# obah/zk-research-implementations

Hardware: AMD Instinct MI355X
Metric: GKR sum-check field-ops/sec + prover ms, 24-var BN254, 1/2/4/8 GPU (higher is better)
Workload: dtype u256 mod p (8x32-bit Montgomery limbs)

## Files before the change

zk-research-implementations_amd/csrc/gkr_plan.hpp:

```cpp
#pragma once
#include <stddef.h>
#include <stdint.h>

#include <vector>

#if defined(__HIPCC__)
#define ZK_PLAN_HD __host__ __device__ __forceinline__
#else
#define ZK_PLAN_HD static inline
#endif

namespace zk {
ZK_PLAN_HD uint64_t tail_region(uint64_t h0, uint32_t m) { return 8 * (h0 - (h0 >> m)); }
ZK_PLAN_HD uint64_t dtail_region(uint64_t Q0, uint32_t s) {
  uint64_t o = 0;
  for (uint32_t t = 0; t < s; ++t) o += 16 * (Q0 >> (2 * t));
  return o;
}
}

namespace zkh {
struct GStep {
  int kind;
  uint32_t i;
  int np;
  uint32_t nd = 0;
  bool dfs = false;
};
enum {
  GS_ROUND0 = 0, GS_SINGLE = 1, GS_DOUBLE = 2, GS_TAIL = 3, GS_DTAIL = 4, GS_D0 = 5, GS_D0T = 6, GS_T32 = 7, GS_T33 = 8,
  GS_HOST = 11
};
inline uint32_t rounds_of(const GStep& st, uint32_t nv) {
  switch (st.kind) {
    case GS_DOUBLE: case GS_D0: case GS_T32: return 2;
    case GS_D0T: case GS_T33: return 3;
    case GS_DTAIL: return 2 * st.nd;
    case GS_TAIL: case GS_HOST: return nv - st.i;
    default: return 1;
  }
}

struct PlanKnobs {
  bool pre = true;
  bool dround = true, d0 = true, d0t = true, dtail = true;
  bool use_tail = true;
  bool cross_ranks = false;
  bool device_fs = false;
  uint64_t dtail_max_quads = 1u << 10, tail_max_pairs = 1u << 15;
  uint32_t host_rounds = 4;
  uint32_t num_cus = 256, t33_oct64_min = 1, mall_order = 0;
};

struct PhasePlan {
  std::vector<GStep> steps;
  uint32_t stop = 0;
  uint32_t host_rounds = 0;
  uint32_t d0t_order = 0;
  uint64_t tail_elems = 0;
  size_t host_tab_bytes = 0;
  bool fslog = false;
  const char* error = nullptr;
};

inline PhasePlan plan_phase(const PlanKnobs& k, uint32_t nv, bool host_ok, uint32_t gather_max) {
  PhasePlan pl;
  std::vector<GStep>& steps = pl.steps;
  const uint64_t L = (uint64_t)1 << nv;
  const bool d0t = k.dround && k.d0t && nv >= 11;
  int nt = -1;
  if (d0t)
    for (int q = 0; 3 + 3 * q + 8 <= (int)nv; ++q) {
      const int R = (int)nv - 3 - 3 * q;
      if (R % 2 == 0 && (R >= 12 || nt < 0)) nt = q;
    }
  const bool d0t_doubles = d0t && nt >= 0;
  const bool d0 = !d0t_doubles && k.dround && k.d0 && nv >= 2 && nv % 2 == 0;
  const bool persistent = k.pre && k.use_tail;
  if (nv >= 1) steps.push_back({d0t_doubles ? GS_D0T : (d0 ? GS_D0 : GS_ROUND0), 0, 0});
  if (d0t_doubles) {
    for (int q = 0; q < nt; ++q) steps.push_back({GS_T33, 3u + 3u * q, 3});
    steps.push_back({GS_T32, 3u + 3u * nt, 3});
  }
  if (k.dround) {
    uint32_t i = d0t_doubles ? 5u + 3u * nt : (d0 ? 2 : 1);
    int np = d0t_doubles || d0 ? 2 : 1;
    if (!d0 && !d0t_doubles) {
      if (nv >= 2) steps.push_back({GS_SINGLE, i++, 0});
      if (nv >= 3 && (nv - 2) % 2 == 1) steps.push_back({GS_SINGLE, i++, 0});
    }
    for (; i + 1 < nv; i += 2, np = 2) steps.push_back({GS_DOUBLE, i, np});
    auto small = [&](const GStep& st) { return st.kind == GS_DOUBLE && (L >> st.i) / 4 <= k.dtail_max_quads; };
    if (host_ok && persistent && k.dtail && !k.cross_ranks && k.host_rounds >= 2) {
      for (uint32_t H = k.host_rounds & ~1u; H >= 2 && pl.host_rounds == 0; H -= 2) {
        size_t e = steps.size();
        uint32_t got = 0;
        while (got < H && e > 0 && steps[e - 1].kind == GS_DOUBLE && steps[e - 1].np == 2) {
          --e;
          got += 2;
        }
        size_t smalls = 0;
        for (size_t q = 0; q < e; ++q) smalls += small(steps[q]);
        if (got == H && smalls >= 2 && e == steps.size() - H / 2) {
          steps.resize(e);
          pl.host_rounds = H;
// ... 78 lines not shown
```

zk-research-implementations_amd/csrc/gkr_rounds.hpp:

```cpp
#pragma once
#include <stddef.h>
#include <stdint.h>
#include <string.h>

#include <vector>

#include "hfield.hpp"
#include "keccak.hpp"

using zk::Fe;

struct zk_transcript {
  zk::Keccak256 h;
};

namespace zkh {
template <class F>
void canon_bytes(const Fe& m, uint8_t out[32]) {
  const Fe c = zk::hfe_from_mont<F>(m);
  memcpy(out, c.v, 32);
}
template <class F>
Fe challenge(zk_transcript* t) {
  uint8_t d[32];
// ... 155 lines not shown
  for (int b = 0; b < 3; ++b) {
    V[b] = fe_zero<F>();
    for (int a = 0; a < 3; ++a)
      V[b] = hfe_add<F>(V[b], hfe_mul<F>(wa[a], hfe_add<F>(T[9 * a + 3 * b], T[9 * a + 3 * b + 1])));
  }
  later_round<F>(s, i0 + 1, V[0], at2w(V[0], V[1], V[2]));
  Fe wb[3];
  wts(s.r, wb);
  Fe Z[3];
  for (int g = 0; g < 3; ++g) {
    uint64_t acc[9] = {0};
    for (int a = 0; a < 3; ++a) {
      uint64_t in[9] = {0};
      for (int b = 0; b < 3; ++b) h64::mac_wide(in, h64::of(wb[b]), h64::of(T[9 * a + 3 * b + g]));
      h64::mac_wide(acc, h64::of(wa[a]), h64::of(wide_to_fe<F>(in)));
    }
    Z[g] = wide_to_fe<F>(acc);
  }
  later_round<F>(s, i0 + 2, Z[0], at2w(Z[0], Z[1], Z[2]));
}

template <class F>
void two_rounds(RoundState& s, uint32_t i0, bool first, const Fe* d) {
  using namespace zk;
  const Fe e0 = hfe_add<F>(d[0], d[2]);
  const Fe e1 = first ? hfe_add<F>(d[4], d[8]) : hfe_sub<F>(s.claim, e0);
  one_round<F>(s, i0, e0, e1, hfe_add<F>(d[5], d[6]));
  const Fe &r = s.r, one = fe_one<F>(), two = hfe_add<F>(one, one);
  const Fe rm1 = hfe_sub<F>(r, one), rm2 = hfe_sub<F>(r, two);
  const Fe L0 = hfe_half<F>(hfe_mul<F>(rm1, rm2));
  const Fe L1 = hfe_sub<F>(fe_zero<F>(), hfe_mul<F>(r, rm2));
  const Fe L2 = hfe_half<F>(hfe_mul<F>(r, rm1));
  auto lag = [&](const Fe& v0, const Fe& v1, const Fe& v2) {
    return hfe_add<F>(hfe_add<F>(hfe_mul<F>(L0, v0), hfe_mul<F>(L1, v1)), hfe_mul<F>(L2, v2));
  };
  const Fe f0 = lag(d[0], d[4], d[5]), f2 = lag(d[3], d[7], d[1]);
  later_round<F>(s, i0 + 1, f0, f2);
}

template <class F>
void eq8_weights(const Fe& rz, const Fe& ra, const Fe& rb, Fe (&e)[8]) {
  using namespace zk;
  Fe ab[4];
  ab[3] = hfe_mul<F>(rz, ra);
  ab[2] = hfe_sub<F>(rz, ab[3]);
  ab[1] = hfe_sub<F>(ra, ab[3]);
  ab[0] = hfe_sub<F>(hfe_sub<F>(fe_one<F>(), rz), ab[1]);
  for (int q = 0; q < 4; ++q) {
    e[2 * q + 1] = hfe_mul<F>(ab[q], rb);
    e[2 * q] = hfe_sub<F>(ab[q], e[2 * q + 1]);
  }
}

template <class F>
void host_rounds(RoundState& s, uint32_t i, uint32_t nv, const uint64_t* raw, FinalVals* fin) {
  const size_t len = (size_t)1 << (nv - i + 2);
  std::vector<Fe> T[4];
  for (int t = 0; t < 4; ++t) {
    const uint64_t* w = raw + (size_t)t * 4 * len;
    T[t].resize(len);
    for (size_t e = 0; e < len; ++e)
      for (int k = 0; k < 4; ++k) {
        const uint64_t x = w[k * len + e];
        T[t][e].v[2 * k] = (uint32_t)x;
        T[t][e].v[2 * k + 1] = (uint32_t)(x >> 32);
      }
  }
  host_fold<F>(T, s.ra);
  host_fold<F>(T, s.rb);
  for (; i < nv; ++i) {
    Fe e0, e2;
    host_round_sums<F>(T, e0, e2);
    later_round<F>(s, i, e0, e2);
    if (i + 1 < nv || fin) host_fold<F>(T, s.r);
  }
  if (fin) {
    for (int t = 0; t < 4; ++t) fin->v[t] = T[t][0];
    fin->ok = true;
  }
}

template <class F>
const char* replay_device_fs(RoundState& s, uint32_t i, const uint32_t (*cf)[8], uint32_t m, const uint32_t* rd) {
  using namespace zk;
  if (m > 3) return "device Fiat-Shamir record corrupt";
  Fe c[3];
  for (uint32_t q = 0; q < 3; ++q) {
    if (q < m) memcpy(c[q].v, cf[q], 32);
    else c[q] = fe_zero<F>();
  }
  const Fe s01 = hfe_add<F>(hfe_add<F>(hfe_add<F>(c[0], c[0]), c[1]), c[2]);
  if (memcmp(s01.v, s.claim.v, 32) != 0) return "device Fiat-Shamir round polynomial does not match the running claim";
  s.claim = absorb_round<F>(s.tr, c, (int)m, s.k0 + i, s.out, s.r);
  if (memcmp(s.r.v, rd, 32) != 0) return "device Fiat-Shamir challenge differs from the host transcript";
  s.drew();
  return nullptr;
}
}
```

zk-research-implementations_amd/csrc/host.hpp:

```cpp
#pragma once
#include <hip/hip_runtime.h>
#include <hip/hip_ext.h>
#include <rccl/rccl.h>

#include <algorithm>
#include <chrono>
#include <cstdio>
#include <cstdlib>
#include <cstring>
#include <memory>
#include <new>
#include <string>
#include <utility>
#include <vector>

#include "../../include/zk_sumcheck.h"
#include "field.hpp"
#include "keccak.hpp"
#include "kernels.hpp"
#include "mfma.hpp"
#include "gkr_plan.hpp"
#include "gkr_rounds.hpp"
#include "fft_plan.hpp"
#include "poly_plan.hpp"
// ... 22 lines not shown
  } while (0)

template <class Fn>
int guarded(Fn&& fn) {
  try {
    fn();
    g_last_error.clear();
    return ZK_OK;
  } catch (const ZkError& e) {
    g_last_error = e.msg;
    return e.code;
  } catch (const std::bad_alloc&) {
    g_last_error = "host allocation failed";
    return ZK_ENOMEM;
  } catch (...) {
    g_last_error = "unknown error";
    return ZK_EDEVICE;
  }
}

inline void require(bool cond, const char* msg) {
  if (!cond) fail(ZK_EINVAL, msg);
}

template <class Fn>
void dispatch(zk_field field, Fn&& fn) {
  switch (field) {
    case ZK_BN254_FR: fn(zk::Bn254Fr{}); break;
    case ZK_BN254_FQ: fn(zk::Bn254Fq{}); break;
    case ZK_BLS12_381_FR: fn(zk::Bls12_381Fr{}); break;
    default: fail(ZK_EINVAL, "unknown field");
  }
}

inline Fe from_zk(const zk_fe& a) {
  Fe r;
  memcpy(r.v, a.limb, 32);
  return r;
}
inline zk_fe to_zk(const Fe& a) {
  zk_fe r;
  memcpy(r.limb, a.v, 32);
  return r;
}

template <class F>
Fe in_mont(zk_repr repr, const zk_fe& a) {
  Fe x = from_zk(a);
  require(zk::fe_is_canonical<F>(x), "field element >= modulus");
  return repr == ZK_REPR_MONTGOMERY ? x : zk::fe_to_mont<F>(x);
}
template <class F>
zk_fe out_repr(zk_repr repr, const Fe& m) {
  return to_zk(repr == ZK_REPR_MONTGOMERY ? m : zk::fe_from_mont<F>(m));
}

}
using namespace zkh;

namespace zkh {
struct DevBuf {
  void* p = nullptr;
  size_t bytes = 0;
  void ensure(size_t b) {
    if (b <= bytes) return;
    if (p) HIPCK(hipFree(p));
    p = nullptr;
    bytes = 0;
    if (hipMalloc(&p, b) != hipSuccess) {
      p = nullptr;
      (void)hipGetLastError();
      fail(ZK_ENOMEM, "hipMalloc of " + std::to_string(b) + " bytes failed");
    }
    bytes = b;
  }
  void release() {
    if (p) (void)hipFree(p);
    p = nullptr;
    bytes = 0;
  }
  Fe* fe(size_t off_elems = 0) const { return reinterpret_cast<Fe*>(p) + off_elems; }
};
struct ScopedBuf {
  DevBuf b;
  ScopedBuf() = default;
  ScopedBuf(const ScopedBuf&) = delete;
  ScopedBuf& operator=(const ScopedBuf&) = delete;
  ~ScopedBuf() { b.release(); }
};

struct FftTables {
  int field = 0;
  uint32_t m = 0;
  bool inverse = false;
  uint32_t log_w = 0, h = 0;
  DevBuf stage_roots, hi, lo, lo_scaled;
  Fe n_inv;
};

enum CommKind { COMM_NONE = 0, COMM_HOST = 1, COMM_RCCL = 2 };
}
using namespace zkh;

struct zk_ctx {
  int device = 0;
  int num_cus = 256;
  hipStream_t stream = nullptr;
  DevBuf work[2];
  DevBuf input;
  DevBuf partials;
  DevBuf tailbuf;
  DevBuf small;
  uint64_t* h_red = nullptr;
  uint32_t tag = 0;
  uint64_t lanes_max_pairs = 1u << 15;
  std::chrono::steady_clock::time_point work_t0;
  bool work_open = false;
  uint32_t timing = 0;
  zk_stats stats{};
  struct Pending {
    int kind;
    hipEvent_t a, b;
    double bytes;
  };
  std::vector<zk_launch> launch_log;
  std::vector<std::pair<hipEvent_t, hipEvent_t>> ev_free;
  std::vector<Pending> pending;
  int rank = 0, world = 1;
  CommKind comm = COMM_NONE;
  zk_allreduce_u64_fn ar = nullptr;
  bool force_coll = false;
  bool prelaunch = true;
  bool host_prelaunch = false;
  bool dround = true;
  int d0 = 3;
  bool d0t = true;
  bool dm = true;
  uint64_t dm_min_quads = 1u << 17;
  bool dtail = true;
  uint64_t dtail_max_quads = 1u << 10;
  uint32_t dtail_blocks = 64;
  uint32_t gather_vars = 10;
  DevBuf gbuf;
  bool t33_pipe = true;
  uint32_t lc_loads = 7;
  uint32_t mall_order = 0;
  uint32_t t33_oct64_min = 1;
  uint32_t host_rounds = 4;
  uint64_t* h_tab = nullptr;
  bool device_fs = false;
  zk::FsLog* h_fslog = nullptr;
  size_t h_tab_bytes = 0;
  bool tail = true;
  bool circuit_dense = false;
  uint32_t circuit_host_lgl = 9;
  uint64_t tail_max_pairs = 1u << 15;
  uint64_t* tail_trace = nullptr;
  uint64_t* block_trace = nullptr;
  int block_trace_step = -1;
  uint32_t grid_cap = 0;
  uint32_t atomic_fanin = 1024;
  uint32_t rtag = 0;
  void* user = nullptr;
  ncclComm_t nccl = nullptr;
  bool peer = false;
  uint64_t* peer_buf = nullptr;
  uint64_t* peer_gbuf = nullptr;
  std::vector<void*> peer_open;
  zk::PeerSlots* d_peer = nullptr;
  uint64_t peer_seq = 0;
  DevBuf msm[19];
  bool msm_balanced = true;
  uint32_t msm_win_task = 4;
  DevBuf scan_tmp[4];
  DevBuf g1_table;
  DevBuf g1_table16;
  uint32_t fft_stages = kFftTileLog;
  DevBuf fft_scratch[2];
  std::vector<std::unique_ptr<FftTables>> fft_tables;
  uint32_t poly_host_max = kPolyHostMaxDefault;
  DevBuf poly_scratch[3];
  uint32_t composed_host_lg = zkc::kComposedHostLgDefault;
  std::vector<zk_wired_circuit*> wired;
};


namespace zkh {
constexpr size_t kSmallBytes = 160 * 1024;
constexpr size_t kBlockTraceMax = 8192;
inline uint64_t* d_red(zk_ctx* c) { return reinterpret_cast<uint64_t*>(c->small.p); }
inline uint32_t* d_flag(zk_ctx* c) { return reinterpret_cast<uint32_t*>(reinterpret_cast<char*>(c->small.p) + 2048); }
inline uint32_t* d_counter(zk_ctx* c) { return reinterpret_cast<uint32_t*>(reinterpret_cast<char*>(c->small.p) + 2560); }
inline uint64_t* d_accum(zk_ctx* c) { return reinterpret_cast<uint64_t*>(reinterpret_cast<char*>(c->small.p) + 4096); }
inline char* d_gather(zk_ctx* c) { return reinterpret_cast<char*>(c->small.p) + 8192; }
constexpr size_t kHostPage = 8192;
inline uint32_t* h_flag(zk_ctx* c) { return reinterpret_cast<uint32_t*>(reinterpret_cast<char*>(c->h_red) + 2048); }
inline zk::RWait* h_rin(zk_ctx* c) { return reinterpret_cast<zk::RWait*>(reinterpret_cast<char*>(c->h_red) + 4096); }
inline uint32_t* h_err(zk_ctx* c) { return reinterpret_cast<uint32_t*>(reinterpret_cast<char*>(c->h_red) + 4160); }
inline zk::RPost* h_rpost(zk_ctx* c) { return reinterpret_cast<zk::RPost*>(reinterpret_cast<char*>(c->h_red) + 6144); }
inline zk::RWait* d_relay(zk_ctx* c) { return reinterpret_cast<zk::RWait*>(reinterpret_cast<char*>(c->small.p) + 6144); }
inline zk::RPost* d_rpost(zk_ctx* c) { return reinterpret_cast<zk::RPost*>(reinterpret_cast<char*>(c->small.p) + 6656); }
static_assert(6656 + sizeof(zk::RPost) <= 8192 && 6144 + sizeof(zk::RPost) <= kHostPage, "relay slot overlaps");

inline void bind(zk_ctx* c) { HIPCK(hipSetDevice(c->device)); }
void wired_release_all(zk_ctx* c);
template <class F>
void eq_table_device(zk_ctx* c, const Fe* pt, uint32_t n, Fe* dst, Fe* tmp);
uint32_t kzg_nvars(const zk_kzg* k);
void check_g1_points(const zk_g1* pts, uint32_t n);

template <class K>
uint32_t grid_for(zk_ctx* c, uint64_t work, K kernel) {
  static thread_local std::vector<std::pair<const void*, int>> cache;
  int per_cu = 0;
  for (auto& e : cache)
// ... 386 lines not shown
    const uint64_t t = (uint64_t)tag << 32;
    for (int i = 0; i < 8; ++i) {
      __atomic_store_n(&s->w[24 + i], t | dig[i], __ATOMIC_RELAXED);
      __atomic_store_n(&s->w[32 + i], t | claim.v[i], __ATOMIC_RELAXED);
    }
    post2(ra, rb, rab, tag);
  }
  ~PostR() {
    if (done || last == 0) return;
    post(zk::fe_zero<zk::Bn254Fr>(), last);
    Fe z[8];
    for (auto& x : z) x = zk::fe_zero<zk::Bn254Fr>();
    post8(z, last);
    (void)hipStreamSynchronize(c->stream);
  }
};

inline bool prelaunch(zk_ctx* c, uint32_t nv) {
  return c->prelaunch && nv > 1 && (c->comm != COMM_HOST || c->host_prelaunch);
}

inline bool use_tail(zk_ctx* c, bool across_ranks) {
  return c->tail && !(across_ranks && multi_rank(c) && (c->comm == COMM_RCCL || c->peer));
}
constexpr size_t kTailRelayBytes = 64 * sizeof(zk::RPost);
inline PlanKnobs plan_knobs(zk_ctx* c, uint32_t nv, bool across_ranks) {
  PlanKnobs k;
  k.pre = prelaunch(c, nv);
  k.dround = c->dround;
  k.d0 = c->d0 > 0;
  k.d0t = c->d0t;
  k.dtail = c->dtail;
  k.use_tail = use_tail(c, across_ranks);
  k.cross_ranks = across_ranks && multi_rank(c);
  k.device_fs = c->device_fs;
  k.dtail_max_quads = c->dtail_max_quads;
  k.tail_max_pairs = c->tail_max_pairs;
  k.host_rounds = c->host_rounds;
  k.num_cus = (uint32_t)c->num_cus;
  k.t33_oct64_min = c->t33_oct64_min;
  k.mall_order = c->mall_order;
  return k;
}

inline void prepare_phase_buffers(zk_ctx* c, const PhasePlan& pl) {
  if (pl.fslog && !c->h_fslog) {
    HIPCK(hipHostMalloc(reinterpret_cast<void**>(&c->h_fslog), 64 * sizeof(zk::FsLog),
                        hipHostMallocMapped | hipHostMallocCoherent));
    memset(c->h_fslog, 0, 64 * sizeof(zk::FsLog));
  }
  if (pl.tail_elems > 0) {
    const size_t had = c->tailbuf.bytes;
    c->tailbuf.ensure(kTailRelayBytes + pl.tail_elems * sizeof(Fe));
    if (c->tailbuf.bytes != had) HIPCK(hipMemset(c->tailbuf.p, 0, kTailRelayBytes));
  }
  if (c->h_tab_bytes < pl.host_tab_bytes) {
    if (c->h_tab) HIPCK(hipHostFree(c->h_tab));
    c->h_tab = nullptr;
    c->h_tab_bytes = 0;
    HIPCK(hipHostMalloc(reinterpret_cast<void**>(&c->h_tab), pl.host_tab_bytes, hipHostMallocMapped | hipHostMallocCoherent));
    c->h_tab_bytes = pl.host_tab_bytes;
  }
}

inline zk::DIn make_din(zk_ctx* c, bool pre, uint32_t& rtag, const Fe& ra, const Fe& rb, const Fe& rab) {
  zk::DIn d{};
  if (pre) {
    d.host = h_rpost(c);
    d.relay = d_rpost(c);
    d.err = h_err(c);
    d.tag = rtag = ++c->rtag;
  } else {
    d.ra = ra;
    d.rb = rb;
    d.rab = rab;
  }
  return d;
}
inline zk::RoundIn make_rin(zk_ctx* c, bool pre, uint32_t& rtag, const Fe& r) {
  zk::RoundIn in{};
  if (pre) {
    in.host = h_rin(c);
    in.relay = d_relay(c);
    in.err = h_err(c);
    in.tag = rtag = ++c->rtag;
  } else {
    in.r = r;
  }
  return in;
}

template <class F>
struct PhaseRun {
  zk_ctx* c;
  const Fe** cur;
  uint32_t nv;
  bool across_ranks, pre;
  const PhasePlan& pl;
  FinalVals* fin;
  RoundState rs;
  std::vector<zk::RoundSink> sinks;
  std::vector<uint32_t> rtags;
  int inbuf;
  PostR post;

  void out_tables(uint64_t size, Fe* nx[4]) {
    const int ob = inbuf == 0 ? 1 : 0;
    Fe* w = c->work[ob].fe();
    for (int t = 0; t < 4; ++t) nx[t] = w + (uint64_t)t * size;
    inbuf = ob;
  }
  void wrote(Fe* const nx[4], const zk::RoundSink& sk, int limbs) {
    for (int t = 0; t < 4; ++t) cur[t] = nx[t];
    enqueue_reduce(c, sk, across_ranks, limbs);
  }

  void enqueue_input(const GStep& st) {
    const uint64_t size = (uint64_t)1 << nv, h = size / 2;
    const zk::RoundSink& sk = sinks[0];
    if (st.kind == GS_ROUND0) {
      const uint32_t grid = grid_for(c, 2 * h, zk::k_gkr_round0<F>);
      launch(c, ZK_K_GKR_ROUND0, 256.0 * h, 6.0 * h, zk::k_gkr_round0<F>, grid, cur[0], cur[1], cur[2], cur[3], h, sk);
      enqueue_reduce(c, sk, across_ranks, 3 * 17);
    } else if (st.kind == GS_D0) {
      const uint64_t Q = size / 4, nch = (Q + 31) / 32;
      const uint32_t res = grid_for(c, nch * zk::kBlock, zk::k_gkr_d0m<F>);
      const uint32_t grid = step_grid(c, res, (nch + 2 * zk::kD0MChunksMax - 1) / (2 * zk::kD0MChunksMax));
      launch(c, ZK_K_GKR_D0, 128.0 * size, 4.5 * size, zk::k_gkr_d0m<F>, grid, cur[0], cur[1], cur[2], cur[3], Q, sk);
      enqueue_reduce(c, sk, across_ranks, zk::kD0Limbs);
    } else {
      const uint64_t O = size / 8, nch = O / 32;
      const auto kern = (c->lc_loads & 1u) ? zk::k_gkr_d0t<F, true> : zk::k_gkr_d0t<F>;
      const uint32_t res = grid_for(c, 2 * nch * zk::kBlock, kern) & ~1u;
      const uint32_t grid = step_grid(c, res, std::max<uint64_t>(2, 2 * ((nch + zk::kD0TChunksMax - 1) / zk::kD0TChunksMax))) & ~1u;
      launch(c, ZK_K_GKR_D0, 128.0 * size, 8.0 * size, kern, grid, cur[0], cur[1], cur[2], cur[3], O, pl.d0t_order, sk);
      enqueue_reduce(c, sk, across_ranks, zk::kD0TLimbs);
    }
  }
  void enqueue_by_three(size_t si) {
    const GStep& st = pl.steps[si];
    const uint64_t size = ((uint64_t)1 << nv) >> st.i;
    const zk::RoundSink& sk = sinks[st.i];
    Fe* nx[4];
    out_tables(size, nx);
    const zk::DIn din = make_din(c, pre, rtags[si], rs.rz, rs.ra, rs.rb);
    if (st.kind == GS_T32) {
      const uint64_t Q = size / 4, nch = Q / zk::kDMQuads;
      const uint32_t res = grid_for(c, nch * zk::kBlock, zk::k_gkr_dm3<F>);
      const uint32_t grid = step_grid(c, res, (nch + zk::kDMChunksMax - 1) / zk::kDMChunksMax);
      launch(c, ZK_K_GKR_DM, 4608.0 * Q, 48.0 * Q, zk::k_gkr_dm3<F>, grid, cur[0], cur[1], cur[2], cur[3], nx[0],
             nx[1], nx[2], nx[3], Q, din, sk);
      return wrote(nx, sk, zk::kDLimbs);
    }
    const uint64_t O = size / 8;
    const bool o64 = O / 64 >= (uint64_t)c->num_cus * c->t33_oct64_min;
// ... 109 lines not shown
    switch (st.kind) {
      case GS_ROUND0: case GS_D0: case GS_D0T: return enqueue_input(st);
      case GS_T32: case GS_T33: return enqueue_by_three(si);
      case GS_TAIL: return enqueue_tail(si);
      case GS_DTAIL: return enqueue_dtail(si);
      case GS_DOUBLE: return enqueue_double(si);
      default: return enqueue_single(si);
    }
  }
  uint32_t last_tag(size_t si) const {
    const GStep& st = pl.steps[si];
    return rtags[si] + (st.kind == GS_TAIL ? nv - st.i - 1 : (st.kind == GS_DTAIL ? st.nd - 1 : 0));
  }

  void single(uint32_t i) {
    Fe s2[2];
    collect_sums<F, 2>(c, sinks[i], across_ranks, 17, s2);
    later_round<F>(rs, i, s2[0], s2[1]);
  }
  void two(uint32_t i0) {
    Fe d[zk::kDCats];
    collect_sums<F, zk::kDCats>(c, sinks[i0], across_ranks, 17, d);
    two_rounds<F>(rs, i0, false, d);
  }
  void three(uint32_t i0, bool first) {
    Fe T[zk::kD0TCats];
    collect_sums<F, zk::kD0TCats>(c, sinks[i0], across_ranks, 9, T, true);
    three_rounds<F>(rs, i0, first, T);
  }
  void post_pair(uint32_t tag) { post.post2(rs.ra, rs.rb, zk::hfe_mul<F>(rs.ra, rs.rb), tag); }
  void dtail(size_t si) {
    const GStep& st = pl.steps[si];
    const uint32_t last = st.i + 2 * (st.nd - 1);
    if (!st.dfs) {
      for (uint32_t d = 0; d < st.nd; ++d) {
        two(st.i + 2 * d);
        if (d + 1 < st.nd) post_pair(rtags[si] + d + 1);
      }
      return;
    }
    wait_flag(c, sinks[last].tag);
    for (uint32_t d = 0; d + 1 < st.nd; ++d) {
      const zk::FsLog& lg = c->h_fslog[d];
      if (__atomic_load_n(&lg.tag, __ATOMIC_ACQUIRE) != rtags[si] + d) fail(ZK_EDEVICE, "device Fiat-Shamir record missing");
      for (int j = 0; j < 2; ++j) {
        if (const char* bad = replay_device_fs<F>(rs, st.i + 2 * d + j, lg.c[j], lg.m[j], lg.r[j])) fail(ZK_EDEVICE, bad);
        c->stats.device_fs_rounds += 1;
      }
    }
    two(last);
  }
  void host(const GStep& st) {
    const auto t0 = std::chrono::steady_clock::now();
    std::vector<uint64_t> raw((size_t)16 << (nv - st.i + 2));
    memcpy(raw.data(), c->h_tab, raw.size() * 8);
    const auto t1 = std::chrono::steady_clock::now();
    host_rounds<F>(rs, st.i, nv, raw.data(), fin);
    if (c->tail_trace)
      fprintf(stderr, "zk host rounds %u..%u: %.2f us (table copy %.2f us)\n", st.i, nv - 1,
              std::chrono::duration<double, std::micro>(std::chrono::steady_clock::now() - t0).count(),
              std::chrono::duration<double, std::micro>(t1 - t0).count());
  }
  uint32_t derive(size_t si) {
    const GStep& st = pl.steps[si];
    switch (st.kind) {
      case GS_ROUND0: {
        Fe s3[3];
        collect_sums<F, 3>(c, sinks[0], across_ranks, 17, s3);
        one_round<F>(rs, 0, s3[0], s3[1], s3[2]);
        return 1;
      }
      case GS_D0: {
        Fe d[zk::kD0Cats];
        collect_sums<F, zk::kD0Cats>(c, sinks[0], across_ranks, 17, d);
        two_rounds<F>(rs, 0, true, d);
        return 2;
      }
      case GS_D0T: case GS_T33: three(st.i, st.kind == GS_D0T); return 3;
      case GS_T32: case GS_DOUBLE: two(st.i); return 2;
      case GS_SINGLE: single(st.i); return 1;
      case GS_TAIL:
        for (uint32_t i = st.i; i < nv; ++i) {
          single(i);
          if (pre && i + 1 < nv) post.post(rs.r, rtags[si] + (i + 1 - st.i));
        }
        return 1;
      case GS_HOST: host(st); return 0;
      default: dtail(si); return 2;
    }
  }
  void hand_on(size_t si) {
    if (!pre || si + 1 >= pl.steps.size()) return;
    const GStep& nx = pl.steps[si + 1];
    const uint32_t tag = rtags[si + 1];
    const Fe z = zk::fe_zero<F>();
    if (nx.kind == GS_HOST) return;
    if (nx.kind == GS_T32 || nx.kind == GS_T33) {
      Fe e[8];
      eq8_weights<F>(rs.rz, rs.ra, rs.rb, e);
      post.post8(e, tag);
    } else if (nx.kind == GS_DTAIL && nx.dfs) {
      const zk::Keccak256& h = rs.tr->h;
      bool fresh = h.fill == 32;
      for (int q = 0; q < 25; ++q) fresh = fresh && h.st[q] == 0;
      if (!fresh) fail(ZK_EINVAL, "internal: device Fiat-Shamir needs a transcript right after a challenge");
      uint32_t dig[8];
      memcpy(dig, h.buf, 32);
      const bool two = nx.np == 2;
      post.post5(two ? rs.ra : z, rs.rb, two ? zk::hfe_mul<F>(rs.ra, rs.rb) : z, dig, rs.claim, tag);
    } else if (nx.kind == GS_DOUBLE || nx.kind == GS_DTAIL) {
// ... 41 lines not shown
      auto pr = [](const char* what, std::vector<double> v) {
        if (v.empty()) return;
        std::sort(v.begin(), v.end());
        fprintf(stderr, "    %-22s min %8.2f  p10 %8.2f  med %8.2f  p90 %8.2f  max %8.2f us (%zu blocks)\n", what, v.front(),
                v[v.size() / 10], v[v.size() / 2], v[v.size() * 9 / 10], v.back(), v.size());
      };
      if (const char* fn = getenv("ZK_DEBUG_BLOCKS_FILE")) {
        if (FILE* f = fopen(fn, "w")) {
          fprintf(f, "block,loop_end,fanin_start,counted_in\n");
          for (size_t b = 0; b < kBlockTraceMax; ++b) {
            const uint64_t* q = c->block_trace + 8 * b;
            if (!q[0] || !q[1] || !q[2]) continue;
            fprintf(f, "%zu,%.2f,%.2f,%.2f\n", b, ((int64_t)q[0] - (int64_t)rr) * 0.01, ((int64_t)q[1] - (int64_t)rr) * 0.01,
                    ((int64_t)q[2] - (int64_t)rr) * 0.01);
          }
          fclose(f);
        }
      }
      pr("r -> loop end", le);
      pr("loop end -> epilogue", ep);
      pr("epilogue -> counted in", ci);
      pr("loop end -> flushed", fl);
      pr("flushed -> words", wd);
      memset(c->block_trace, 0, kBlockTraceMax * 64);
    }
  }
  const uint64_t* T = c->tail_trace;
  if (ns > 0 && steps.back().kind == GS_TAIL) {
    const uint32_t nr = nv - steps.back().i;
    for (uint32_t m = 0; m < nr; ++m)
      fprintf(stderr, "zk tail round %2u: wait r %6.2f us, fold+eval %6.2f, fan-in %6.2f, publish %6.2f, hand-off to next r %6.2f\n",
              m, (T[m * 8 + 1] - T[m * 8]) * 0.01, (T[m * 8 + 2] - T[m * 8 + 1]) * 0.01, (T[m * 8 + 3] - T[m * 8 + 2]) * 0.01,
              (T[m * 8 + 4] - T[m * 8 + 3]) * 0.01, m + 1 < nr ? (T[m * 8 + 9] - T[m * 8 + 4]) * 0.01 : 0.0);
  }
  const size_t sdt = ns > 0 && steps.back().kind == GS_HOST ? ns - 2 : ns - 1;
  if (ns > 0 && steps[sdt].kind == GS_DTAIL) {
    const uint32_t nd = steps[sdt].nd;
    for (uint32_t m = 0; m < nd; ++m)
      fprintf(stderr, "zk dtail step %u: wait r %6.2f us, fold+eval %6.2f, limb sums %6.2f, fan-in %6.2f, publish %6.2f, hand-off to next r %6.2f\n",
              m, (T[m * 8 + 1] - T[m * 8]) * 0.01, (T[m * 8 + 2] - T[m * 8 + 1]) * 0.01, (T[m * 8 + 3] - T[m * 8 + 2]) * 0.01,
              (T[m * 8 + 4] - T[m * 8 + 3]) * 0.01, (T[m * 8 + 5] - T[m * 8 + 4]) * 0.01,
              m + 1 < nd ? (T[m * 8 + 9] - T[m * 8 + 5]) * 0.01 : 0.0);
    for (uint32_t m = 0; m < nd; ++m)
      fprintf(stderr, "zk dtail step %u fold+eval: constants %6.2f us, loop %6.2f, store drain %6.2f\n", m,
              (T[m * 8 + 6] - T[m * 8 + 1]) * 0.01, (T[m * 8 + 7] - T[m * 8 + 6]) * 0.01, (T[m * 8 + 2] - T[m * 8 + 7]) * 0.01);
  }
}

template <class F>
void gkr_phase(zk_ctx* c, const Fe* cur[4], uint32_t nv, uint32_t k0, bool across_ranks, zk_transcript* tr,
               GkrOut& out, Fe& claim, Fe& r, uint32_t& pend, bool host_ok = false, uint32_t gather_max = 0,
               uint32_t* stop = nullptr, FinalVals* fin = nullptr) {
  if (fin) fin->ok = false;
  const PlanKnobs knobs = plan_knobs(c, nv, across_ranks);
  const PhasePlan plan = plan_phase(knobs, nv, host_ok, gather_max);
  if (plan.error) fail(ZK_EINVAL, plan.error);
  if (stop) *stop = plan.stop;
  prepare_phase_buffers(c, plan);
  const size_t ns = plan.steps.size();
  const bool pre = knobs.pre;
  const Fe z = zk::fe_zero<F>();
  PhaseRun<F> run{c, cur, nv, across_ranks, pre, plan, fin, RoundState{tr, out, claim, r, k0, z, z, z},
                  std::vector<zk::RoundSink>(nv), std::vector<uint32_t>(ns, 0), -1, PostR{c}};
  if (pre) {
    const auto t0 = std::chrono::steady_clock::now();
    for (size_t si = 0; si < ns; ++si) {
      run.enqueue(si);
      run.post.last = run.last_tag(si);
    }
    if (getenv("ZK_DEBUG_ENQUEUE"))
      fprintf(stderr, "zk: enqueued %zu steps (%u rounds) in %.1f us\n", ns, nv,
              std::chrono::duration<double, std::micro>(std::chrono::steady_clock::now() - t0).count());
  }
  for (size_t si = 0; si < ns; ++si) {
    if (!pre) run.enqueue(si);
    pend = run.derive(si);
    run.hand_on(si);
  }
  run.post.done = true;
  if (c->tail_trace) run.report();
}

template <class F>
void gkr_prove_device(zk_ctx* c, const Fe* const dT[4], uint32_t nloc, bool sharded, zk_transcript* tr, GkrOut& out) {
  const int G = sharded ? c->world : 1;
  uint32_t lg = 0;
  while ((1 << lg) < G) ++lg;
  const uint32_t n = nloc + lg;
  out.coeffs.assign(3 * (size_t)n, zk::fe_zero<F>());
  out.ncoeffs.assign(n, 0);
  out.challenges.assign(n, zk::fe_zero<F>());
  if (n == 0) return;
  ensure_partials(c, nloc);
  __atomic_store_n(h_err(c), 0u, __ATOMIC_RELAXED);
  const uint64_t Lloc = (uint64_t)1 << nloc;
  const uint64_t wmax = std::max<uint64_t>(Lloc / 2, (uint64_t)G);
  c->work[0].ensure(4 * wmax * 32);
  c->work[1].ensure(4 * std::max<uint64_t>(wmax / 2, 1) * 32);
  const Fe* cur[4] = {dT[0], dT[1], dT[2], dT[3]};
  Fe claim = zk::fe_zero<F>(), r = zk::fe_zero<F>();
  uint32_t pend = 0;
  uint32_t stop = nloc;
  const bool coll = sharded && (lg > 0 || (c->force_coll && c->comm != COMM_NONE));
  gkr_phase<F>(c, cur, nloc, 0, sharded, tr, out, claim, r, pend, !coll,
               coll ? c->gather_vars : 0, &stop);
  if (!coll) {
    sync(c);
    return;
  }
  if (stop < nloc) {
    const uint32_t T = nloc - stop;
    const uint64_t Tn = (uint64_t)1 << T;
    const uint64_t sz = (uint64_t)1 << (T + pend);
    const size_t scratch = (size_t)4 * sz, onehot = (size_t)G * 4 * Tn, global = (size_t)4 * G * Tn;
    c->gbuf.ensure((scratch + onehot + global) * sizeof(Fe));
    Fe* sc = reinterpret_cast<Fe*>(c->gbuf.p);
    Fe* oh = sc + scratch;
    Fe* gl = oh + onehot;
    const bool via_peer = c->peer && T <= zk::kPeerGatherMaxT;
    if (c->comm != COMM_RCCL && !via_peer) HIPCK(hipMemsetAsync(oh, 0, onehot * sizeof(Fe), c->stream));
    Fe* slot = oh + (size_t)c->rank * 4 * Tn;
    if (pend == 0) {
      for (int t = 0; t < 4; ++t) HIPCK(hipMemcpyAsync(slot + t * Tn, cur[t], Tn * 32, hipMemcpyDeviceToDevice, c->stream));
    }
    for (uint32_t j = 0; j < pend; ++j) {
      const uint64_t half = sz >> (j + 1);
      Fe* dst = j + 1 == pend ? slot : sc + (j & 1 ? 2 * sz : 0);
      const uint64_t dstride = j + 1 == pend ? Tn : half;
      const Fe& rj = out.challenges[stop - pend + j];
      launch(c, ZK_K_FOLD, 4 * half * 96.0, 4.0 * half, zk::k_fold4<F>, grid_for(c, half, zk::k_fold4<F>), cur[0], cur[1],
             cur[2], cur[3], dst, dst + dstride, dst + 2 * dstride, dst + 3 * dstride, half, rj);
      for (int t = 0; t < 4; ++t) cur[t] = dst + t * dstride;
    }
    const Fe* gsrc = oh;
    if (via_peer) {
      const uint64_t cap = (uint64_t)4 * ((uint64_t)1 << zk::kPeerGatherMaxT);
      launch_peer_gather(c, slot, 4 * Tn * 4);
      c->stats.collectives += 1;
      if (cap != 4 * Tn) {
        HIPCK(hipMemcpy2DAsync(oh, 4 * Tn * sizeof(Fe), c->peer_gbuf, cap * sizeof(Fe), 4 * Tn * sizeof(Fe), (size_t)G,
                               hipMemcpyDeviceToDevice, c->stream));
      } else {
        gsrc = reinterpret_cast<const Fe*>(c->peer_gbuf);
      }
    } else if (c->comm == COMM_RCCL) {
      CollTimer ct(c, 4.0 * Tn * 32);
      NCCLCK(ncclAllGather(slot, oh, (size_t)4 * Tn * 4, ncclUint64, c->nccl, c->stream));
      c->stats.collectives += 1;
    } else {
      std::vector<uint64_t> w(onehot * 4);
      HIPCK(hipMemcpyAsync(w.data(), oh, onehot * sizeof(Fe), hipMemcpyDeviceToHost, c->stream));
      sync(c);
      allreduce_host(c, w.data(), w.size());
      HIPCK(hipMemcpyAsync(oh, w.data(), onehot * sizeof(Fe), hipMemcpyHostToDevice, c->stream));
      sync(c);
    }
    launch(c, ZK_K_FOLD, global * 64.0, 0.0, zk::k_interleave<F>, grid_for(c, global, zk::k_interleave<F>), gsrc, gl,
           Tn, (uint32_t)G);
    const Fe* gcur[4] = {gl, gl + G * Tn, gl + 2 * G * Tn, gl + 3 * G * Tn};
    gkr_phase<F>(c, gcur, T + lg, stop, false, tr, out, claim, r, pend, true);
// ... 173 lines not shown
```

zk-research-implementations_amd/csrc/zk_sumcheck.hip:

```cpp
#include "host.hpp"

using namespace zkh;

extern "C" {

uint32_t zk_abi_version(void) { return ZK_ABI_VERSION; }
const char* zk_last_error(void) { return g_last_error.c_str(); }

int zk_ctx_create(int device, zk_ctx** out) {
  return guarded([&] {
    require(out != nullptr, "out is null");
    *out = nullptr;
    int ndev = 0;
    if (hipGetDeviceCount(&ndev) != hipSuccess || ndev == 0) {
      (void)hipGetLastError();
      fail(ZK_EDEVICE, "no HIP device available (the prover has no CPU fallback)");
    }
    require(device >= 0 && device < ndev, "device index out of range");
    hipDeviceProp_t prop;
    HIPCK(hipGetDeviceProperties(&prop, device));
    if (std::string(prop.gcnArchName).rfind("gfx950", 0) != 0)
      fail(ZK_EDEVICE, std::string("kernels are built for gfx950, device is ") + prop.gcnArchName);
    auto* c = new zk_ctx();
    c->device = device;
    if (const char* e = getenv("ZK_LANES_MAX_PAIRS")) c->lanes_max_pairs = strtoull(e, nullptr, 0);
    if (const char* e = getenv("ZK_FORCE_COLLECTIVES")) c->force_coll = atoi(e) != 0;
    if (const char* e = getenv("ZK_PRELAUNCH")) c->prelaunch = atoi(e) != 0;
    if (const char* e = getenv("ZK_HOST_PRELAUNCH")) c->host_prelaunch = atoi(e) != 0;
    if (const char* e = getenv("ZK_TAIL")) c->tail = atoi(e) != 0;
    if (const char* e = getenv("ZK_DROUND")) c->dround = atoi(e) != 0;
    if (const char* e = getenv("ZK_DTAIL")) c->dtail = atoi(e) != 0;
    if (const char* e = getenv("ZK_DM")) c->dm = atoi(e) != 0;
    if (const char* e = getenv("ZK_D0T")) c->d0t = atoi(e) != 0;
    if (const char* e = getenv("ZK_DM_MIN_QUADS")) c->dm_min_quads = strtoull(e, nullptr, 0);
    if (const char* e = getenv("ZK_D0")) c->d0 = atoi(e);
    if (const char* e = getenv("ZK_CIRCUIT_DENSE")) c->circuit_dense = atoi(e) != 0;
    if (const char* e = getenv("ZK_CIRCUIT_HOST_LGL")) c->circuit_host_lgl = (uint32_t)strtoul(e, nullptr, 0);
    if (const char* e = getenv("ZK_DTAIL_MAX_QUADS")) c->dtail_max_quads = strtoull(e, nullptr, 0);
    if (const char* e = getenv("ZK_GRID_CAP")) c->grid_cap = (uint32_t)strtoul(e, nullptr, 0);
    if (const char* e = getenv("ZK_FFT_STAGES")) c->fft_stages = fft_stage_cap(strtol(e, nullptr, 0));
    if (const char* e = getenv("ZK_POLY_HOST_MAX")) c->poly_host_max = poly_host_max(*e ? strtol(e, nullptr, 0) : -1);
    if (const char* e = getenv("ZK_ATOMIC_FANIN")) c->atomic_fanin = (uint32_t)strtoul(e, nullptr, 0);
    if (const char* e = getenv("ZK_DTAIL_BLOCKS")) c->dtail_blocks = (uint32_t)strtoul(e, nullptr, 0);
    if (const char* e = getenv("ZK_GATHER_VARS")) c->gather_vars = (uint32_t)strtoul(e, nullptr, 0);
    if (const char* e = getenv("ZK_T33_PIPE")) c->t33_pipe = atoi(e) != 0;
    if (const char* e = getenv("ZK_MSM_BALANCED")) c->msm_balanced = atoi(e) != 0;
    if (const char* e = getenv("ZK_MSM_WIN_TASK")) c->msm_win_task = std::max<uint32_t>(2u, (uint32_t)strtoul(e, nullptr, 0));
    if (const char* e = getenv("ZK_T33_OCT64_MIN")) c->t33_oct64_min = (uint32_t)strtoul(e, nullptr, 0);
    if (const char* e = getenv("ZK_LC_LOADS")) c->lc_loads = (uint32_t)strtoul(e, nullptr, 0) & 7u;
    if (const char* e = getenv("ZK_MALL_ORDER")) c->mall_order = std::min<uint32_t>((uint32_t)strtoul(e, nullptr, 0), 2u);
    if (const char* e = getenv("ZK_HOST_ROUNDS"))
      c->host_rounds = std::min<uint32_t>((uint32_t)strtoul(e, nullptr, 0), 8u);
    if (const char* e = getenv("ZK_COMPOSED_HOST_LG"))
      c->composed_host_lg = std::min<uint32_t>((uint32_t)strtoul(e, nullptr, 0), zkc::kComposedHostLgMax);
    if (const char* e = getenv("ZK_DEVICE_FS")) c->device_fs = atoi(e) != 0;
    if (const char* e = getenv("ZK_TAIL_MAX_PAIRS")) c->tail_max_pairs = strtoull(e, nullptr, 0);
    c->num_cus = prop.multiProcessorCount;
    try {
      bind(c);
      HIPCK(hipStreamCreateWithFlags(&c->stream, hipStreamNonBlocking));
      c->small.ensure(kSmallBytes);
      HIPCK(hipMemset(c->small.p, 0, kSmallBytes));
      HIPCK(hipHostMalloc(reinterpret_cast<void**>(&c->h_red), kHostPage, hipHostMallocMapped | hipHostMallocCoherent));
      memset(c->h_red, 0, kHostPage);
      if (getenv("ZK_DEBUG_TAIL")) {
        HIPCK(hipHostMalloc(reinterpret_cast<void**>(&c->tail_trace), 1024 * 8, hipHostMallocMapped | hipHostMallocCoherent));
        memset(c->tail_trace, 0, 1024 * 8);
        if (const char* b = getenv("ZK_DEBUG_BLOCKS")) {
          c->block_trace_step = atoi(b);
          HIPCK(hipHostMalloc(reinterpret_cast<void**>(&c->block_trace), zkh::kBlockTraceMax * 64,
                              hipHostMallocMapped | hipHostMallocCoherent));
          memset(c->block_trace, 0, zkh::kBlockTraceMax * 64);
        }
      }
    } catch (...) {
      zk_ctx_destroy(c);
      throw;
    }
    *out = c;
  });
}

void zk_ctx_destroy(zk_ctx* c) {
  if (!c) return;
  (void)hipSetDevice(c->device);
  if (c->stream) (void)hipStreamSynchronize(c->stream);
  if (c->nccl) (void)ncclCommDestroy(c->nccl);
  wired_release_all(c);
  for (auto& p : c->pending) c->ev_free.push_back({p.a, p.b});
  for (auto& e : c->ev_free) {
    (void)hipEventDestroy(e.first);
    (void)hipEventDestroy(e.second);
  }
  c->work[0].release();
  c->work[1].release();
  c->input.release();
  c->partials.release();
  c->tailbuf.release();
  if (c->tail_trace) (void)hipHostFree(c->tail_trace);
  if (c->block_trace) (void)hipHostFree(c->block_trace);
  c->small.release();
  c->gbuf.release();
  for (auto& b : c->msm) b.release();
  for (auto& b : c->scan_tmp) b.release();
  c->g1_table.release();
  c->g1_table16.release();
  for (auto& b : c->fft_scratch) b.release();
  for (auto& b : c->poly_scratch) b.release();
  for (auto& t : c->fft_tables) {
// ... 323 lines not shown
    require(claimed_sum && transcript && out_verified && out_final_claimed_sum && out_challenges, "null argument");
    require(nrounds == 0 || (coeffs && ncoeffs), "null argument");
    dispatch(field, [&](auto f) {
      using F = decltype(f);
      using namespace zk;
      Fe claim = in_mont<F>(repr, *claimed_sum);
      const Fe zero = fe_zero<F>(), one = fe_one<F>();
      for (uint32_t k = 0; k < nrounds; ++k) {
        require(ncoeffs[k] <= 3, "round polynomial has more than 3 coefficients");
        Fe cf[3];
        const int m = ncoeffs[k];
        for (int i = 0; i < m; ++i) cf[i] = in_mont<F>(repr, coeffs[3 * k + i]);
        auto eval = [&](const Fe& x) {
          Fe s = zero, xp = one;
          for (int i = 0; i < m; ++i) {
            s = fe_add<F>(s, fe_mul<F>(cf[i], xp));
            xp = fe_mul<F>(xp, x);
          }
          return s;
        };
        if (!fe_eq<F>(fe_add<F>(eval(zero), eval(one)), claim)) {
          *out_verified = 0;
          *out_final_claimed_sum = out_repr<F>(repr, zero);
          out_challenges[0] = out_repr<F>(repr, zero);
          return;
        }
        absorb<F>(transcript, cf, (size_t)m);
        const Fe r = challenge<F>(transcript);
        out_challenges[k] = out_repr<F>(repr, r);
        claim = eval(r);
      }
      *out_verified = 1;
      *out_final_claimed_sum = out_repr<F>(repr, claim);
    });
  });
}

int zk_dev_alloc(zk_ctx* c, size_t bytes, void** out) {
  return guarded([&] {
    require(c && out, "null argument");
    bind(c);
    *out = nullptr;
    if (hipMalloc(out, bytes ? bytes : 1) != hipSuccess) {
      (void)hipGetLastError();
      *out = nullptr;
      fail(ZK_ENOMEM, "hipMalloc failed");
    }
  });
}
int zk_dev_free(zk_ctx* c, void* p) {
  return guarded([&] {
    require(c, "null ctx");
    bind(c);
    if (p) HIPCK(hipFree(p));
  });
}
int zk_dev_upload(zk_ctx* c, zk_field field, zk_repr repr, const zk_fe* host, size_t n, void* dev) {
  return guarded([&] {
    require(c && (n == 0 || (host && dev)), "null argument");
    bind(c);
    dispatch(field, [&](auto f) {
      using F = decltype(f);
      upload<F>(c, repr, host, n, reinterpret_cast<Fe*>(dev));
    });
  });
}
int zk_dev_download(zk_ctx* c, zk_field field, zk_repr repr, const void* dev, size_t n, zk_fe* host) {
  return guarded([&] {
    require(c && (n == 0 || (host && dev)), "null argument");
    bind(c);
    dispatch(field, [&](auto f) {
      using F = decltype(f);
      download<F>(c, repr, reinterpret_cast<const Fe*>(dev), n, host);
    });
  });
}
int zk_dev_synth_fill(zk_ctx* c, zk_field field, void* dev, uint64_t count, uint64_t seed, uint32_t table,
                      uint64_t index0, uint64_t stride) {
  return guarded([&] {
    require(c && (dev || count == 0), "null argument");
    bind(c);
    dispatch(field, [&](auto f) {
      using F = decltype(f);
      const uint64_t key = zk::splitmix64(zk::splitmix64(seed) + table);
      const uint32_t grid = grid_for(c, count, zk::k_synth<F>);
      launch(c, ZK_K_SYNTH, 32.0 * count, (double)count, zk::k_synth<F>, grid, reinterpret_cast<Fe*>(dev), count, key, index0, stride);
      sync(c);
    });
  });
}
int zk_dev_mle_partial_evaluate(zk_ctx* c, zk_field field, const void* d_in, uint32_t nvars, uint32_t bit,
                                zk_repr repr, const zk_fe* value, void* d_out) {
  return guarded([&] {
    require(c && d_in && d_out && value, "null argument");
    require(nvars >= 1 && bit < nvars, "pair_points underflow panics");
    require(d_in != d_out, "d_out may not alias d_in");
    bind(c);
    dispatch(field, [&](auto f) {
      using F = decltype(f);
      const Fe r = in_mont<F>(repr, *value);
      const uint64_t half = (uint64_t)1 << (nvars - 1);
      const uint32_t grid = grid_for(c, half, zk::k_fold<F>);
      const uint32_t s = nvars - 1 - bit;
      launch(c, ZK_K_FOLD, 96.0 * half, (double)half, zk::k_fold<F>, grid, reinterpret_cast<const Fe*>(d_in), reinterpret_cast<Fe*>(d_out), half, s, r);
      sync(c);
    });
// ... 158 lines not shown
```

Before: 552.6 billion.

## Cache phase plans, reuse host scratch, and fuse host two-variable fold

Phase plans and their buffer preparation are now cached per context, keyed on nv, host_ok, gather_max and the knob set, so planning is not redone on every call. Round sinks, rtags and the host-round tables are kept in context-owned vectors instead of being reallocated each time. The first two host folds are merged into one weighted four-way pass with a wide multiply-accumulate that reduces once, and the tail memset becomes async. The last sync is skipped when nothing is pending, and extra synchronizes are added before frees to stay safe now that memset work is queued on the stream.

```diff
diff --git a/zk-research-implementations_amd/csrc/gkr_plan.hpp b/zk-research-implementations_amd/csrc/gkr_plan.hpp
--- a/zk-research-implementations_amd/csrc/gkr_plan.hpp
+++ b/zk-research-implementations_amd/csrc/gkr_plan.hpp
@@ -51,6 +51,14 @@
   uint32_t host_rounds = 4;
   uint32_t num_cus = 256, t33_oct64_min = 1, mall_order = 0;
 };
+
+inline bool same_knobs(const PlanKnobs& a, const PlanKnobs& b) {
+  return a.pre == b.pre && a.dround == b.dround && a.d0 == b.d0 && a.d0t == b.d0t && a.dtail == b.dtail &&
+         a.use_tail == b.use_tail && a.cross_ranks == b.cross_ranks && a.device_fs == b.device_fs &&
+         a.dtail_max_quads == b.dtail_max_quads && a.tail_max_pairs == b.tail_max_pairs &&
+         a.host_rounds == b.host_rounds && a.num_cus == b.num_cus && a.t33_oct64_min == b.t33_oct64_min &&
+         a.mall_order == b.mall_order;
+}
 
 struct PhasePlan {
   std::vector<GStep> steps;
diff --git a/zk-research-implementations_amd/csrc/gkr_rounds.hpp b/zk-research-implementations_amd/csrc/gkr_rounds.hpp
--- a/zk-research-implementations_amd/csrc/gkr_rounds.hpp
+++ b/zk-research-implementations_amd/csrc/gkr_rounds.hpp
@@ -231,22 +231,33 @@
   }
 }
 
-template <class F>
-void host_rounds(RoundState& s, uint32_t i, uint32_t nv, const uint64_t* raw, FinalVals* fin) {
-  const size_t len = (size_t)1 << (nv - i + 2);
+struct HostRoundScratch {
   std::vector<Fe> T[4];
+  std::vector<uint64_t> raw;
+};
+template <class F>
+void host_rounds(RoundState& s, uint32_t i, uint32_t nv, const uint64_t* raw, FinalVals* fin, HostRoundScratch& hs) {
+  using namespace zk;
+  const size_t len = (size_t)1 << (nv - i + 2), q = len / 4;
+  std::vector<Fe> (&T)[4] = hs.T;
+  const Fe w11 = hfe_mul<F>(s.ra, s.rb);
+  const Fe w10 = hfe_sub<F>(s.ra, w11);
+  const Fe w01 = hfe_sub<F>(s.rb, w11);
+  const Fe w00 = hfe_sub<F>(hfe_sub<F>(fe_one<F>(), s.ra), w01);
+  const h64::V wt[4] = {h64::of(w00), h64::of(w01), h64::of(w10), h64::of(w11)};
   for (int t = 0; t < 4; ++t) {
     const uint64_t* w = raw + (size_t)t * 4 * len;
-    T[t].resize(len);
-    for (size_t e = 0; e < len; ++e)
-      for (int k = 0; k < 4; ++k) {
-        const uint64_t x = w[k * len + e];
-        T[t][e].v[2 * k] = (uint32_t)x;
-        T[t][e].v[2 * k + 1] = (uint32_t)(x >> 32);
+    T[t].resize(q);
+    for (size_t j = 0; j < q; ++j) {
+      uint64_t acc[9] = {0};
+      for (int c = 0; c < 4; ++c) {
+        const size_t e = j + c * q;
+        const h64::V x = {{w[e], w[len + e], w[2 * len + e], w[3 * len + e]}};
+        h64::mac_wide(acc, wt[c], x);
       }
-  }
-  host_fold<F>(T, s.ra);
-  host_fold<F>(T, s.rb);
+      T[t][j] = wide_to_fe<F>(acc);
+    }
+  }
   for (; i < nv; ++i) {
     Fe e0, e2;
     host_round_sums<F>(T, e0, e2);
@@ -257,6 +268,11 @@
     for (int t = 0; t < 4; ++t) fin->v[t] = T[t][0];
     fin->ok = true;
   }
+}
+template <class F>
+void host_rounds(RoundState& s, uint32_t i, uint32_t nv, const uint64_t* raw, FinalVals* fin) {
+  HostRoundScratch hs;
+  host_rounds<F>(s, i, nv, raw, fin, hs);
 }
 
 template <class F>
diff --git a/zk-research-implementations_amd/csrc/host.hpp b/zk-research-implementations_amd/csrc/host.hpp
--- a/zk-research-implementations_amd/csrc/host.hpp
+++ b/zk-research-implementations_amd/csrc/host.hpp
@@ -98,7 +98,7 @@
 }
 template <class F>
 zk_fe out_repr(zk_repr repr, const Fe& m) {
-  return to_zk(repr == ZK_REPR_MONTGOMERY ? m : zk::fe_from_mont<F>(m));
+  return to_zk(repr == ZK_REPR_MONTGOMERY ? m : zk::hfe_from_mont<F>(m));
 }
 
 }
@@ -110,6 +110,7 @@
   size_t bytes = 0;
   void ensure(size_t b) {
     if (b <= bytes) return;
+    if (p) HIPCK(hipDeviceSynchronize());
     if (p) HIPCK(hipFree(p));
     p = nullptr;
     bytes = 0;
@@ -121,6 +122,7 @@
     bytes = b;
   }
   void release() {
+    if (p) (void)hipDeviceSynchronize();
     if (p) (void)hipFree(p);
     p = nullptr;
     bytes = 0;
@@ -207,6 +209,19 @@
   uint32_t grid_cap = 0;
   uint32_t atomic_fanin = 1024;
   uint32_t rtag = 0;
+  struct PlannedPhase {
+    uint32_t nv;
+    bool host_ok;
+    uint32_t gather_max;
+    PlanKnobs knobs;
+    PhasePlan plan;
+    bool buffers = false;
+  };
+  std::vector<std::unique_ptr<PlannedPhase>> plans;
+  std::vector<zk::RoundSink> run_sinks;
+  std::vector<uint32_t> run_rtags;
+  HostRoundScratch host_scratch;
+  bool debug_enqueue = false;
   void* user = nullptr;
   ncclComm_t nccl = nullptr;
   bool peer = false;
@@ -699,15 +714,37 @@
   if (pl.tail_elems > 0) {
     const size_t had = c->tailbuf.bytes;
     c->tailbuf.ensure(kTailRelayBytes + pl.tail_elems * sizeof(Fe));
-    if (c->tailbuf.bytes != had) HIPCK(hipMemset(c->tailbuf.p, 0, kTailRelayBytes));
+    if (c->tailbuf.bytes != had)
+      HIPCK(hipMemsetAsync(c->tailbuf.p, 0, kTailRelayBytes, c->stream));
   }
   if (c->h_tab_bytes < pl.host_tab_bytes) {
+    if (c->h_tab) HIPCK(hipStreamSynchronize(c->stream));
     if (c->h_tab) HIPCK(hipHostFree(c->h_tab));
     c->h_tab = nullptr;
     c->h_tab_bytes = 0;
     HIPCK(hipHostMalloc(reinterpret_cast<void**>(&c->h_tab), pl.host_tab_bytes, hipHostMallocMapped | hipHostMallocCoherent));
     c->h_tab_bytes = pl.host_tab_bytes;
   }
+}
+
+constexpr size_t kPlansMax = 128;
+inline const PhasePlan& planned_phase(zk_ctx* c, uint32_t nv, bool across_ranks, bool host_ok, uint32_t gather_max) {
+  const PlanKnobs knobs = plan_knobs(c, nv, across_ranks);
+  zk_ctx::PlannedPhase* e = nullptr;
+  for (auto& p : c->plans)
+    if (p->nv == nv && p->host_ok == host_ok && p->gather_max == gather_max && same_knobs(p->knobs, knobs)) e = p.get();
+  if (!e) {
+    if (c->plans.size() >= kPlansMax) c->plans.clear();
+    c->plans.push_back(std::make_unique<zk_ctx::PlannedPhase>(
+        zk_ctx::PlannedPhase{nv, host_ok, gather_max, knobs, plan_phase(knobs, nv, host_ok, gather_max)}));
+    e = c->plans.back().get();
+  }
+  if (e->plan.error) fail(ZK_EINVAL, e->plan.error);
+  if (!e->buffers) {
+    prepare_phase_buffers(c, e->plan);
+    e->buffers = true;
+  }
+  return e->plan;
 }
 
 inline zk::DIn make_din(zk_ctx* c, bool pre, uint32_t& rtag, const Fe& ra, const Fe& rb, const Fe& rab) {
@@ -746,8 +783,8 @@
   const PhasePlan& pl;
   FinalVals* fin;
   RoundState rs;
-  std::vector<zk::RoundSink> sinks;
-  std::vector<uint32_t> rtags;
+  std::vector<zk::RoundSink>& sinks;
+  std::vector<uint32_t>& rtags;
   int inbuf;
   PostR post;
 
@@ -963,10 +1000,11 @@
   }
   void host(const GStep& st) {
     const auto t0 = std::chrono::steady_clock::now();
-    std::vector<uint64_t> raw((size_t)16 << (nv - st.i + 2));
+    std::vector<uint64_t>& raw = c->host_scratch.raw;
+    raw.resize((size_t)16 << (nv - st.i + 2));
     memcpy(raw.data(), c->h_tab, raw.size() * 8);
     const auto t1 = std::chrono::steady_clock::now();
-    host_rounds<F>(rs, st.i, nv, raw.data(), fin);
+    host_rounds<F>(rs, st.i, nv, raw.data(), fin, c->host_scratch);
     if (c->tail_trace)
       fprintf(stderr, "zk host rounds %u..%u: %.2f us (table copy %.2f us)\n", st.i, nv - 1,
               std::chrono::duration<double, std::micro>(std::chrono::steady_clock::now() - t0).count(),
@@ -1114,23 +1152,22 @@
                GkrOut& out, Fe& claim, Fe& r, uint32_t& pend, bool host_ok = false, uint32_t gather_max = 0,
                uint32_t* stop = nullptr, FinalVals* fin = nullptr) {
   if (fin) fin->ok = false;
-  const PlanKnobs knobs = plan_knobs(c, nv, across_ranks);
-  const PhasePlan plan = plan_phase(knobs, nv, host_ok, gather_max);
-  if (plan.error) fail(ZK_EINVAL, plan.error);
+  const PhasePlan& plan = planned_phase(c, nv, across_ranks, host_ok, gather_max);
   if (stop) *stop = plan.stop;
-  prepare_phase_buffers(c, plan);
   const size_t ns = plan.steps.size();
-  const bool pre = knobs.pre;
+  const bool pre = prelaunch(c, nv);
   const Fe z = zk::fe_zero<F>();
+  c->run_sinks.assign(nv, zk::RoundSink{});
+  c->run_rtags.assign(ns, 0);
   PhaseRun<F> run{c, cur, nv, across_ranks, pre, plan, fin, RoundState{tr, out, claim, r, k0, z, z, z},
-                  std::vector<zk::RoundSink>(nv), std::vector<uint32_t>(ns, 0), -1, PostR{c}};
+                  c->run_sinks, c->run_rtags, -1, PostR{c}};
   if (pre) {
     const auto t0 = std::chrono::steady_clock::now();
     for (size_t si = 0; si < ns; ++si) {
       run.enqueue(si);
       run.post.last = run.last_tag(si);
     }
-    if (getenv("ZK_DEBUG_ENQUEUE"))
+    if (c->debug_enqueue)
       fprintf(stderr, "zk: enqueued %zu steps (%u rounds) in %.1f us\n", ns, nv,
               std::chrono::duration<double, std::micro>(std::chrono::steady_clock::now() - t0).count());
   }
@@ -1167,7 +1204,10 @@
   gkr_phase<F>(c, cur, nloc, 0, sharded, tr, out, claim, r, pend, !coll,
                coll ? c->gather_vars : 0, &stop);
   if (!coll) {
-    sync(c);
+    if (c->pending.empty())
+      c->work_open = false;
+    else
+      sync(c);
     return;
   }
   if (stop < nloc) {
diff --git a/zk-research-implementations_amd/csrc/zk_sumcheck.hip b/zk-research-implementations_amd/csrc/zk_sumcheck.hip
--- a/zk-research-implementations_amd/csrc/zk_sumcheck.hip
+++ b/zk-research-implementations_amd/csrc/zk_sumcheck.hip
@@ -55,6 +55,7 @@
       c->composed_host_lg = std::min<uint32_t>((uint32_t)strtoul(e, nullptr, 0), zkc::kComposedHostLgMax);
     if (const char* e = getenv("ZK_DEVICE_FS")) c->device_fs = atoi(e) != 0;
     if (const char* e = getenv("ZK_TAIL_MAX_PAIRS")) c->tail_max_pairs = strtoull(e, nullptr, 0);
+    c->debug_enqueue = getenv("ZK_DEBUG_ENQUEUE") != nullptr;
     c->num_cus = prop.multiProcessorCount;
     try {
       bind(c);
@@ -484,6 +485,7 @@
   return guarded([&] {
     require(c, "null ctx");
     bind(c);
+    if (p && c->stream) HIPCK(hipStreamSynchronize(c->stream));
     if (p) HIPCK(hipFree(p));
   });
 }
```

New measurement: 547.1 billion. Within noise of the previous version (-1.0%).
